# nunofonseca/fastq_utils

Measured on AMD Instinct MI355X. Metric: Mreads/s validated (fastq_info, 150bp), higher is better.
Workload: dtype u8

## Files before the change

fastq_utils_amd/csrc/fqg_mark_pack.h:

```cpp
#pragma once
#include <stdint.h>

#if defined(__HIPCC__) || defined(__CUDACC__)
#define FQG_PACK_HD __host__ __device__ inline
#else
#define FQG_PACK_HD inline
#endif

namespace fqg {

FQG_PACK_HD uint32_t udot4_u8(uint32_t a, uint32_t b, uint32_t c) {
#if defined(__HIP_DEVICE_COMPILE__)
  return __builtin_amdgcn_udot4(a, b, c, false);
#else
  for (int i = 0; i < 4; ++i) c += ((a >> (8 * i)) & 0xFFu) * ((b >> (8 * i)) & 0xFFu);
  return c;
#endif
}

FQG_PACK_HD uint32_t as_computed(uint32_t x) {
#if defined(__HIP_DEVICE_COMPILE__)
  asm("" : "+v"(x));
#endif
  return x;
}

FQG_PACK_HD uint32_t mark_pair(uint32_t m0, uint32_t m1) {
  return udot4_u8(m1, 0x80402010u, udot4_u8(m0, 0x08040201u, 0u));
}

FQG_PACK_HD uint32_t pack_marks32(uint32_t m0, uint32_t m1, uint32_t m2, uint32_t m3, uint32_t m4, uint32_t m5, uint32_t m6,
                                  uint32_t m7) {
  const uint32_t a = as_computed((mark_pair(m2, m3) << 8) | mark_pair(m0, m1));
  const uint32_t b = as_computed((mark_pair(m6, m7) << 8) | mark_pair(m4, m5));
  return (b << 9) | (a >> 7);
}

}
```

fastq_utils_amd/csrc/fqg_stream_kernels.hip:

```cpp
#include "fqg_device.h"
#include "fqg_type_spans.h"
#include "fqg_mark_pack.h"
#include "fqg_part_steps.h"
#include "fqg_line_window.h"

namespace fqg {

constexpr uint32_t kH = 0x80808080u;

__device__ __forceinline__ uint32_t pack_marks16(uint32_t m0, uint32_t m1, uint32_t m2, uint32_t m3) {
  uint32_t lo = __builtin_amdgcn_udot4(m0, 0x08040201u, 0u, false);
  lo = __builtin_amdgcn_udot4(m1, 0x80402010u, lo, false);
  uint32_t hi = __builtin_amdgcn_udot4(m2, 0x08040201u, 0u, false);
  hi = __builtin_amdgcn_udot4(m3, 0x80402010u, hi, false);
  return (lo >> 7) | (hi << 1);
}

__device__ __forceinline__ uint32_t nl_marks7(uint32_t w, uint32_t& bad) {
  const uint32_t x = w ^ 0x0A0A0A0Au;
  const uint32_t t = kH - x;
  const uint32_t c = t + 0x1F1F1F1Fu;
  bad = __builtin_amdgcn_bitop3_b32(bad, c, t, 0xF4);
  return t & kH;
}
__device__ __forceinline__ uint32_t or3(uint32_t a, uint32_t b, uint32_t c) { return __builtin_amdgcn_bitop3_b32(a, b, c, 0xFE); }

__device__ __forceinline__ uint32_t in_vgpr(uint32_t x) {
  uint32_t v;
  asm volatile("v_mov_b32 %0, %1" : "=v"(v) : "s"(x));
  return v;
}

__device__ __forceinline__ uint32_t not_acgtn7(uint32_t w) {
  const uint32_t want = __builtin_amdgcn_perm(0x474E7F54u, 0x437F417Fu, w & 0x07070707u);
  return ((w ^ want) + 0x7F7F7F7Fu) & kH;
}

__device__ __forceinline__ uint32_t in_range7(uint32_t w, uint32_t lob, uint32_t hihb, uint32_t kh = kH) {
  return ((w | kH) - lob) & (hihb - w) & kh;
}
__device__ __forceinline__ uint32_t in_range7a(uint32_t w, uint32_t lo_add, uint32_t hihb, uint32_t kh) {
  return (w + lo_add) & (hihb - w) & kh;
}

constexpr uint32_t kBootMax = 64u << 10;
constexpr int kBootBlock = 1024;
__global__ __launch_bounds__(kBootBlock) void k_stream_boot(const uint8_t* __restrict__ img, uint32_t span,
                                                            CallState* __restrict__ cs) {
  constexpr int kBootWaves = kBootBlock / kWave;
  __shared__ uint32_t s_cnt[kBootWaves];
  __shared__ __attribute__((aligned(16))) uint8_t s_img[kBootMax];
  const int lane = lane_id(), wv = threadIdx.x >> 6;
  const uint32_t part = span / kBootWaves;
  for (uint32_t o = threadIdx.x * 16u; o < span; o += kBootBlock * 16u)
    *reinterpret_cast<uint4*>(s_img + o) = *reinterpret_cast<const uint4*>(img + o);
  __syncthreads();
  const uint8_t* p = s_img + (uint64_t)wv * part;
  uint32_t cnt = 0;
  for (uint32_t o = lane; o < part; o += kWave) cnt += (p[o] == '\n');
  cnt = wave_sum(cnt);
  if (lane == 0) s_cnt[wv] = cnt;
  __syncthreads();
  uint32_t before = 0, total = 0;
  for (int w = 0; w < kBootWaves; ++w) {
    if (w < wv) before += s_cnt[w];
    total += s_cnt[w];
  }
  const uint32_t limit = total & ~3u;
  if (threadIdx.x == 0) cs->boot_lines = total;
  uint32_t line = before, qmin = 255, qmax = 0;
  for (uint32_t o = 0; o < part; o += kWave) {
    const uint32_t c = o + lane < part ? (uint32_t)p[o + lane] : 0u;
    const uint64_t bal = __ballot(o + lane < part && c == '\n');
    const uint32_t mine = line + (uint32_t)__builtin_popcountll(bal & ((1ull << lane) - 1ull));
    if ((mine & 3u) == 3u && mine < limit && c != '\n' && o + lane < part) {
      qmin = c < qmin ? c : qmin;
      qmax = c > qmax ? c : qmax;
    }
    line += (uint32_t)__builtin_popcountll(bal);
  }
#pragma unroll
  for (int d = 32; d > 0; d >>= 1) {
    const uint32_t a = __shfl_xor(qmin, d, 64), b = __shfl_xor(qmax, d, 64);
    qmin = a < qmin ? a : qmin;
    qmax = b > qmax ? b : qmax;
  }
  if (lane == 0 && qmin <= qmax) {
    atomicMin(&cs->boot_qmin, qmin);
    atomicMax(&cs->boot_qmax, qmax);
    atomicMin(&cs->qmin_byte, qmin);
    atomicMax(&cs->qmax_byte, qmax);
  }
}

struct StreamOut {
  uint32_t* counts;
  uint32_t* cinfo;
  uint16_t* stage;
  unsigned long long* queue;
  unsigned long long queue_cap;
};

__device__ __forceinline__ void queue_suspect(const StreamOut& o, CallState* cs, uint64_t pos) {
  if (__hip_atomic_load(&cs->queue_count, __ATOMIC_RELAXED, __HIP_MEMORY_SCOPE_AGENT) > o.queue_cap) return;
  const unsigned long long at = atomicAdd(&cs->queue_count, 1ull);
  if (at < o.queue_cap) o.queue[at] = pos;
}

constexpr int kHalves = 2;
constexpr int kLaneBytes = 32;
constexpr int kHalfBytes = kWave * kLaneBytes;

struct Piece32 {
  uint4 a, b;
};

constexpr uint32_t kCopyFront = 16, kCopyBack = 64;
constexpr uint32_t kCopyRow = kCopyFront + kChunkBytes + kCopyBack;

__device__ __forceinline__ uint32_t stage_entry(uint32_t ent, uint32_t c1) {
  return ent | ((c1 == '@' ? kClsAt : (c1 == '+' ? kClsPlus : 0u)) << 12);
}

template <uint32_t ABL>
__device__ __forceinline__ void stage_chunk(const uint8_t* __restrict__ img, uint64_t n, uint64_t cb, uint32_t chunk,
                                            const uint32_t (&nl)[kHalves], const uint32_t (&nl2)[kHalves],
                                            const uint32_t (&ex)[kHalves], uint32_t tot, bool fits,
                                            uint16_t* __restrict__ slots, const uint8_t* __restrict__ copy,
                                            uint32_t tail, uint16_t* __restrict__ stage, bool interior) {
  const int lane = lane_id();
#pragma unroll
  for (int k = 0; k < kHalves; ++k) {
    uint32_t m = nl[k], r = ex[k];
    const uint32_t at = (uint32_t)k * kHalfBytes + (uint32_t)lane * kLaneBytes;
    if (fits) {
      while (m) {
        const uint32_t j = (uint32_t)__builtin_ctz(m);
        m &= m - 1;
        slots[r] = (uint16_t)((__builtin_amdgcn_ubfe(nl2[k], j, 1u) << 14) | as_computed(at | j));
        ++r;
      }
      continue;
    }
    while (m) {
      const uint32_t j = (uint32_t)__builtin_ctz(m);
      m &= m - 1;
      if (r < (uint32_t)kStageCap) slots[r] = (uint16_t)((at + j) | (((nl2[k] >> j) & 1u) << 14));
      ++r;
    }
  }
  __builtin_amdgcn_wave_barrier();
  uint16_t* dst = stage + (uint64_t)chunk * kStageCap;
  for (uint32_t i = lane; i < tot; i += kWave) {
    const uint32_t ent = slots[i];
    const uint32_t o = (ent & 0xFFFu) + 1;
    uint32_t c1 = 0;
    if (!(ABL & 4u)) {
      if (interior) c1 = o < (uint32_t)kChunkBytes ? (uint32_t)copy[o] : (tail & 0xFFu);
      else c1 = cb + o < n ? (uint32_t)img[cb + o] : 0u;
    }
    dst[i] = (uint16_t)stage_entry(ent, c1);
  }
}

template <int NAMES>
struct Pass1Lds {
  uint16_t slots[kBlock / kWave][kStageCap];
  __attribute__((aligned(16))) uint8_t copy[kBlock / kWave][NAMES ? kCopyRow : (uint32_t)kChunkBytes];
};
template <uint32_t ABL, int NAMES>
__device__ __forceinline__ void stream_pass1_body(const uint8_t* __restrict__ img, uint64_t n, uint32_t n_chunks, const StreamOut& o,
                                                  CallState* __restrict__ cs, const NameCapture& nc, uint32_t block,
                                                  Pass1Lds<NAMES>& lds) {
  static_assert(kHalves == 2 && kHalves * kHalfBytes == kChunkBytes, "one packed scan covers the two slices");
  static_assert(NAMES == 0 || !(ABL & 7u), "the name capture needs the speculation, the staged entries and the copy");
  auto& s_slots = lds.slots;
  auto& s_copy = lds.copy;
  const int lane = lane_id(), wv = __builtin_amdgcn_readfirstlane((int)(threadIdx.x >> 6));
  uint8_t* const copy = s_copy[wv] + (NAMES ? kCopyFront : 0u);
  const uint32_t chunk = block * (kBlock / kWave) + wv;
  if (chunk >= n_chunks) return;
  const uint64_t cb = (uint64_t)chunk * kChunkBytes;
  const uint64_t wb = cb + (uint64_t)lane * kLaneBytes;
  const bool interior = cb + kChunkBytes + 4 <= n;
  uint32_t nl[kHalves], ex[kHalves];
  Piece32 v[kHalves];
  uint32_t flags = 0;

  uint32_t tail = 0;
  uint32_t prev = '\n';
  const uint32_t boot_lo = cs->boot_qmin, boot_hi = cs->boot_qmax;
  if (interior) {
    tail = *reinterpret_cast<const uint32_t*>(img + cb + kChunkBytes);
    if (NAMES && chunk) prev = *reinterpret_cast<const uint32_t*>(img + cb - 4) >> 24;
#pragma unroll
    for (int k = 0; k < kHalves; ++k) {
      v[k].a = *reinterpret_cast<const uint4*>(img + wb + (uint64_t)k * kHalfBytes);
      v[k].b = *reinterpret_cast<const uint4*>(img + wb + (uint64_t)k * kHalfBytes + 16);
    }
    if (!(ABL & 6u)) {
#pragma unroll
      for (int k = 0; k < kHalves; ++k) {
        *reinterpret_cast<uint4*>(&copy[k * kHalfBytes + lane * kLaneBytes]) = v[k].a;
        *reinterpret_cast<uint4*>(&copy[k * kHalfBytes + lane * kLaneBytes + 16]) = v[k].b;
      }
    }
    uint32_t hiacc = 0, badacc = 0;
#pragma unroll
    for (int k = 0; k < kHalves; ++k) {
      hiacc = or3(or3(or3(or3(hiacc, v[k].a.x, v[k].a.y), v[k].a.z, v[k].a.w), v[k].b.x, v[k].b.y), v[k].b.z, v[k].b.w);
      nl[k] = pack_marks32(nl_marks7(v[k].a.x, badacc), nl_marks7(v[k].a.y, badacc), nl_marks7(v[k].a.z, badacc), nl_marks7(v[k].a.w, badacc),
                           nl_marks7(v[k].b.x, badacc), nl_marks7(v[k].b.y, badacc), nl_marks7(v[k].b.z, badacc), nl_marks7(v[k].b.w, badacc));
    }
    const bool high = __ballot((hiacc & kH) != 0) != 0;
    const bool ctrl = __ballot((badacc & kH) != 0) != 0;
    if (high) flags |= kFlagHigh;
    if (ctrl && !high) {
      uint32_t nul = 0, cr = 0;
#pragma unroll
      for (int k = 0; k < kHalves; ++k) {
        const uint32_t w[8] = {v[k].a.x, v[k].a.y, v[k].a.z, v[k].a.w, v[k].b.x, v[k].b.y, v[k].b.z, v[k].b.w};
#pragma unroll
        for (int j = 0; j < 8; ++j) {
          nul |= eq_bytes(w[j], 0u);
          cr |= eq_bytes(w[j], 0x0D0D0D0Du);
        }
      }
      if (__ballot(nul != 0)) flags |= kFlagNul;
      if (__ballot(cr != 0)) flags |= kFlagCr;
    }
  } else {
    uint32_t bad = 0;
#pragma unroll
    for (int k = 0; k < kHalves; ++k) {
      const uint64_t off = wb + (uint64_t)k * kHalfBytes;
      nl[k] = 0;
      v[k].a = v[k].b = make_uint4(0, 0, 0, 0);
      for (uint64_t i = off; i < n && i < off + kLaneBytes; ++i) {
        const uint32_t c = img[i];
        if (c == '\n') nl[k] |= 1u << (i - off);
        else if (c == 0u) bad |= kFlagNul;
        else if (c == '\r') bad |= kFlagCr;
        else if (c >= 0x80u) bad |= kFlagHigh;
      }
    }
    if (__ballot((bad & kFlagNul) != 0)) flags |= kFlagNul;
    if (__ballot((bad & kFlagCr) != 0)) flags |= kFlagCr;
    if (__ballot((bad & kFlagHigh) != 0)) flags |= kFlagHigh;
  }

  const uint32_t c01 = __popc(nl[0]) | (__popc(nl[1]) << 16);
  const uint32_t s01 = wave_scan_incl_dpp(c01);
  const uint32_t t01 = __builtin_amdgcn_readlane(s01, 63);
  const uint32_t total = (t01 & 0xFFFFu) + (t01 >> 16);
  ex[0] = (s01 & 0xFFFFu) - (c01 & 0xFFFFu);
  ex[1] = (t01 & 0xFFFFu) + (s01 >> 16) - (c01 >> 16);
  if (total > (uint32_t)kStageCap) flags |= kFlagStageOverflow;

  uint32_t tail_nl = 0;
  if (interior) {
    tail_nl = ((tail & 0xFFu) == '\n' ? 1u : 0u) | (((tail >> 8) & 0xFFu) == '\n' ? 2u : 0u);
  } else {
    for (uint64_t i = 0; i < 2; ++i)
      if (cb + kChunkBytes + i < n && img[cb + kChunkBytes + i] == '\n') tail_nl |= 1u << i;
  }
  uint32_t nl2[kHalves], cand[kHalves];
#pragma unroll
  for (int k = 0; k < kHalves; ++k) {
    uint32_t nxt = dpp0<0x130, 0xf, 0xf>(nl[k]);
    const uint32_t first_next = (uint32_t)__builtin_amdgcn_readlane(nl[k + 1 < kHalves ? k + 1 : k], 0);
    if (lane == 63) nxt = k + 1 < kHalves ? first_next : tail_nl;
    const uint32_t n1 = __builtin_amdgcn_alignbit(nxt, nl[k], 1);
    nl2[k] = __builtin_amdgcn_alignbit(nxt, nl[k], 2);
    cand[k] = nl[k] & nl2[k] & ~n1;
  }

  const uint32_t tot = total < (uint32_t)kStageCap ? total : (uint32_t)kStageCap;

  uint32_t info = kInfoUnknown;
  bool found = false;
  uint32_t t0 = 0;
  if (!(ABL & 1u) && interior && !(flags & kFlagHigh)) {
#pragma unroll
    for (int k = 0; k < kHalves; ++k) {
      const uint64_t bal = __ballot(cand[k] != 0);
      if (!found && bal) {
        const int l = __builtin_ctzll(bal);
        const uint32_t cl = (uint32_t)__builtin_amdgcn_readlane(cand[k], l);
        const uint32_t nll = (uint32_t)__builtin_amdgcn_readlane(nl[k], l);
        const uint32_t exl = (uint32_t)__builtin_amdgcn_readlane(ex[k], l);
        const uint32_t j = (uint32_t)__builtin_ctz(cl);
        const uint32_t a = exl + __popc(nll & ((1u << j) - 1u));
        t0 = (1u - a) & 3u;
        found = true;
      }
    }
    uint32_t M1[kHalves], M3[kHalves];
    bool dense = false;
    if (found) {
      uint32_t over = 0;
#pragma unroll
      for (int k = 0; k < kHalves; ++k) over |= type_spans32(nl[k], t0 + ex[k], M1[k], M3[k]);
      dense = __ballot(over != 0) != 0;
    }
    if (found && !dense) {
      info = t0;
      uint32_t lo = boot_lo, hi = boot_hi;
      if (lo > hi || lo > 127u) {
        lo = 127u;
        hi = 0u;
      }
      const uint32_t hihb_s = ((hi & 0x7Fu) | 0x80u) * 0x01010101u;
      const uint32_t lo_add = in_vgpr((0x80u - lo) * 0x01010101u), hihb = in_vgpr(hihb_s), khv = in_vgpr(kH);
      QRange q{0x00FF00FFu, 0x00FF00FFu, 0u, 0u};
      bool any_viol = false;
#pragma unroll
      for (int k = 0; k < kHalves; ++k) {
        const uint4 &a = v[k].a, &b = v[k].b;
        const uint32_t inv = pack_marks32(not_acgtn7(a.x), not_acgtn7(a.y), not_acgtn7(a.z), not_acgtn7(a.w), not_acgtn7(b.x), not_acgtn7(b.y),
                                          not_acgtn7(b.z), not_acgtn7(b.w));
        const uint32_t bad = (ABL & 8u) ? 0u : inv & M1[k];
        if (bad) queue_suspect(o, cs, wb + (uint64_t)k * kHalfBytes + (uint32_t)__builtin_ctz(bad));
        const uint32_t okq = pack_marks32(in_range7a(a.x, lo_add, hihb, khv), in_range7a(a.y, lo_add, hihb, khv), in_range7a(a.z, lo_add, hihb, khv),
                                          in_range7a(a.w, lo_add, hihb, khv), in_range7a(b.x, lo_add, hihb, khv), in_range7a(b.y, lo_add, hihb, khv),
                                          in_range7a(b.z, lo_add, hihb, khv), in_range7a(b.w, lo_add, hihb, khv));
        const uint32_t qm = (ABL & 16u) ? 0u : M3[k];
        if (__ballot((qm & ~okq) != 0)) {
          any_viol = true;
          qrange_accum(a, qm & 0xFFFFu, q);
          qrange_accum(b, qm >> 16, q);
        }
      }
      if (any_viol) {
        uint32_t qmin = pk_min_u16(q.mn_e, q.mn_o), qmax = pk_max_u16(q.mx_e, q.mx_o);
        qmin = (qmin & 0xFFFFu) < (qmin >> 16) ? (qmin & 0xFFFFu) : (qmin >> 16);
        qmax = (qmax & 0xFFFFu) > (qmax >> 16) ? (qmax & 0xFFFFu) : (qmax >> 16);
#pragma unroll
        for (int d = 32; d > 0; d >>= 1) {
          const uint32_t x = __shfl_xor(qmin, d, 64), y = __shfl_xor(qmax, d, 64);
          qmin = x < qmin ? x : qmin;
          qmax = y > qmax ? y : qmax;
        }
        if (qmin <= qmax) info |= kInfoRange | ((qmin & 0xFFu) << 8) | ((qmax & 0xFFu) << 16);
      }
    } else if (total == 0) {
      info = kInfoOneLine;
      uint32_t lo = boot_lo, hi = boot_hi;
      if (lo > hi || lo > 127u) {
        lo = 127u;
        hi = 0u;
      }
      const uint32_t lob = lo * 0x01010101u, hihb = ((hi & 0x7Fu) | 0x80u) * 0x01010101u;
      uint32_t not_base = 0, outside = 0;
#pragma unroll
      for (int k = 0; k < kHalves; ++k) {
        const uint32_t w[8] = {v[k].a.x, v[k].a.y, v[k].a.z, v[k].a.w, v[k].b.x, v[k].b.y, v[k].b.z, v[k].b.w};
#pragma unroll
        for (int j = 0; j < 8; ++j) {
          not_base |= not_acgtn7(w[j]);
          outside |= ~in_range7(w[j], lob, hihb) & kH;
        }
      }
      if (__ballot(not_base != 0)) info |= kInfoNotBases;
      if (__ballot(outside != 0)) {
        QRange q{0x00FF00FFu, 0x00FF00FFu, 0u, 0u};
#pragma unroll
        for (int k = 0; k < kHalves; ++k) {
          qrange_accum(v[k].a, 0xFFFFu, q);
          qrange_accum(v[k].b, 0xFFFFu, q);
        }
        uint32_t qmin = pk_min_u16(q.mn_e, q.mn_o), qmax = pk_max_u16(q.mx_e, q.mx_o);
        qmin = (qmin & 0xFFFFu) < (qmin >> 16) ? (qmin & 0xFFFFu) : (qmin >> 16);
        qmax = (qmax & 0xFFFFu) > (qmax >> 16) ? (qmax & 0xFFFFu) : (qmax >> 16);
#pragma unroll
        for (int d = 32; d > 0; d >>= 1) {
          const uint32_t x = __shfl_xor(qmin, d, 64), y = __shfl_xor(qmax, d, 64);
          qmin = x < qmin ? x : qmin;
          qmax = y > qmax ? y : qmax;
        }
        if (qmin <= qmax) info |= kInfoRange | ((qmin & 0xFFu) << 8) | ((qmax & 0xFFu) << 16);
      }
    }
  }

  if (!(ABL & 2u)) {
    stage_chunk<ABL>(img, n, cb, chunk, nl, nl2, ex, tot, total <= (uint32_t)kStageCap, s_slots[wv], copy, tail, o.stage, interior);
  }
  if constexpr (NAMES == 2) {
    uint32_t hc = kNoCapture;
    if (found && total <= (uint32_t)kStageCap) {
      hc = 0;
      const uint16_t* slots = s_slots[wv];
      const bool first_is_start = prev == '\n';
      uint32_t v0 = (0u - t0) & 3u;
      if (v0 == 0u && !first_is_start) v0 = 4u;
      const uint32_t sub = (uint32_t)lane & 3u, q = (uint32_t)lane >> 2;
      const bool casava = nc.fmt == FQG_NAME_CASAVA18;
      const uint32_t pe_cut = (nc.fmt == FQG_NAME_DEFAULT && nc.is_pe) ? 1u : 0u;
      for (uint32_t base = 0; v0 + 4u * base <= tot; base += kWave / 4) {
        const uint32_t j = base + q, vv = v0 + 4u * j;
        bool is_hdr = vv <= tot;
        uint32_t at = 0;
        if (is_hdr && vv > 0) {
          at = (slots[vv - 1] & 0xFFFu) + 1u;
          is_hdr = at < (uint32_t)kChunkBytes;
        }
        hc += (uint32_t)__builtin_popcountll(__ballot(is_hdr && sub == 0u));
        if (is_hdr && j < nc.K) {
// ... 69 lines not shown
          part += oth;
          if (sub == 0u) {
            typedef unsigned long long u64x2 __attribute__((ext_vector_type(2)));
            u64x2 dg;
            dg.x = name_fin(name_seed(nlen) + part);
            dg.y = (unsigned long long)(nlen | (acct << 10) | (vv << 20) | (at_sign ? kDigestAt : 0u) | (ok ? kDigestOk : 0u));
            *reinterpret_cast<u64x2*>(nc.recs + ((uint64_t)chunk * nc.K + j) * kDigestWords) = dg;
          }
        }
      }
      if (hc >= kNoCapture) hc = kNoCapture - 1u;
    }
    if (lane == 0) nc.hcount[chunk] = (uint16_t)hc;
  }
  if constexpr (NAMES == 1) {
    uint32_t hc = kNoCapture;
    if (found && total <= (uint32_t)kStageCap) {
      hc = 0;
      const uint16_t* slots = s_slots[wv];
      const bool first_is_start = prev == '\n';
      for (uint32_t base = 0; base <= tot; base += kWave) {
        const uint32_t vv = base + (uint32_t)lane;
        bool is_hdr = vv <= tot && ((t0 + vv) & 3u) == 0u && (vv > 0 || first_is_start);
        uint32_t at = 0;
        if (is_hdr && vv > 0) {
          at = (slots[vv - 1] & 0xFFFu) + 1u;
          is_hdr = at < (uint32_t)kChunkBytes;
        }
        const unsigned long long hm = __ballot(is_hdr);
        const uint32_t j = hc + (uint32_t)__builtin_popcountll(hm & ((1ull << lane) - 1ull));
        hc += (uint32_t)__builtin_popcountll(hm);
        if (is_hdr && j < nc.K) {
          bool end_known = vv < tot, real = false;
          uint32_t len = (end_known ? (uint32_t)(slots[vv] & 0xFFFu) : (uint32_t)kChunkBytes) - at;
          unsigned long long w[kNameRecWords];
          if (end_known || cb + at + kNameRecText + 1 > n) {
#pragma unroll
            for (uint32_t k = 0; k < kNameRecWords; ++k) __builtin_memcpy(&w[k], copy + at + 8u * k - 3u, 8);
          } else {
            const uint8_t* g = img + cb + at - 3u;
            unsigned long long nlm[kNameRecWords];
#pragma unroll
            for (uint32_t k = 0; k < kNameRecWords; ++k) {
              __builtin_memcpy(&w[k], g + 8u * k, 8);
              const unsigned long long y = w[k] ^ 0x0A0A0A0A0A0A0A0Aull;
              nlm[k] = ~(((y & 0x7F7F7F7F7F7F7F7Full) + 0x7F7F7F7F7F7F7F7Full) | y | 0x7F7F7F7F7F7F7F7Full);
            }
            nlm[0] &= ~0xFFFFFFull;
            real = true;
            len = kNameRecText + 1;
#pragma unroll
            for (int k = (int)kNameRecWords - 1; k >= 0; --k)
              if (nlm[k]) {
                len = 8u * (uint32_t)k + ((uint32_t)__builtin_ctzll(nlm[k]) >> 3) - 3u;
                end_known = true;
              }
          }
          len = len > 1023u ? 1023u : len;
          const uint32_t meta = len | (vv << 10) | (end_known ? 1u << 19 : 0u) | (((w[0] >> 24) & 0xFFu) == '@' ? 1u << 20 : 0u) |
                                (real ? 1u << 21 : 0u);
          w[0] = (w[0] & 0xFFFFFFFF00000000ull) | meta;
          typedef unsigned long long u64x2 __attribute__((ext_vector_type(2)));
          u64x2* dst = reinterpret_cast<u64x2*>(nc.recs + ((uint64_t)chunk * nc.K + j) * kNameRecWords);
#pragma unroll
          for (uint32_t k = 0; k < kNameRecWords / 2; ++k) {
            u64x2 x;
            x.x = w[2 * k];
            x.y = w[2 * k + 1];
            dst[k] = x;
          }
        }
      }
      if (hc >= kNoCapture) hc = kNoCapture - 1u;
    }
    if (lane == 0) nc.hcount[chunk] = (uint16_t)hc;
  }
  if (lane == 0) {
    o.counts[chunk] = total;
    o.cinfo[chunk] = info;
    if (flags) atomicOr(&cs->flags, flags);
  }
}

template <uint32_t ABL, int NAMES = 0>
__global__ __launch_bounds__(kBlock) void k_stream_pass1(const uint8_t* __restrict__ img, uint64_t n,
                                                         uint32_t n_chunks, StreamOut o,
                                                         CallState* __restrict__ cs, NameCapture nc = NameCapture{}) {
  __shared__ Pass1Lds<NAMES> lds;
  stream_pass1_body<ABL, NAMES>(img, n, n_chunks, o, cs, nc, blockIdx.x, lds);
}

struct ChunkRanks {
  const uint32_t* counts;
  const uint32_t* local;
  const unsigned long long* span_excl;
  uint32_t n_chunks;
  __device__ __forceinline__ uint64_t rank0(uint32_t c) const { return span_excl[c / kScanSpan] + local[c]; }
};

__global__ __launch_bounds__(kBlock) void k_stream_chunks(ChunkRanks cr, const uint32_t* __restrict__ cinfo, uint64_t limit,
                                                          uint32_t* __restrict__ redo, CallState* __restrict__ cs) {
  const uint32_t c = blockIdx.x * kBlock + threadIdx.x;
  const int lane = lane_id();
  bool again = false;
  if (c < cr.n_chunks) {
    const uint64_t rank0 = cr.rank0(c);
    const uint32_t cnt = cr.counts[c], info = cinfo[c];
    if (rank0 < limit) {
      if (chunk_info_redo(info, (uint32_t)rank0) || rank0 + cnt >= limit) again = true;
      else if (chunk_info_range(info, (uint32_t)rank0)) {
        const uint32_t qlo = (info >> 8) & 0xFFu, qhi = (info >> 16) & 0xFFu;
        if (qlo < __atomic_load_n(&cs->qmin_byte, __ATOMIC_RELAXED)) atomicMin(&cs->qmin_byte, qlo);
        if (qhi > __atomic_load_n(&cs->qmax_byte, __ATOMIC_RELAXED)) atomicMax(&cs->qmax_byte, qhi);
      }
    }
  }
  __shared__ uint32_t s_cnt[kBlock / kWave], s_base;
  const unsigned long long am = __ballot(again);
  const int wv = (int)(threadIdx.x >> 6);
  if (lane == 0) s_cnt[wv] = (uint32_t)__builtin_popcountll(am);
  __syncthreads();
  if (threadIdx.x == 0) {
    uint32_t tot = 0;
#pragma unroll
    for (int w = 0; w < kBlock / kWave; ++w) tot += s_cnt[w];
    s_base = tot ? atomicAdd(&cs->redo_count, tot) : 0u;
  }
  __syncthreads();
  if (again) {
    uint32_t at = s_base + (uint32_t)__builtin_popcountll(am & ((1ull << lane) - 1ull));
    for (int w = 0; w < wv; ++w) at += s_cnt[w];
    if (at < cr.n_chunks) redo[at] = c;
  }
}

__device__ __forceinline__ uint32_t chunk_of_rank(const ChunkRanks& cr, uint64_t R, uint32_t g) {
  const uint32_t n = cr.n_chunks;
  if (g >= n) g = n - 1;
  uint32_t lo, hi, step = 1;
  if (cr.rank0(g) <= R) {
    lo = g;
    for (;;) {
      const uint32_t t = lo + step;
      if (t >= n) {
        hi = n;
        break;
      }
      if (cr.rank0(t) <= R) {
        lo = t;
        step <<= 1;
      } else {
        hi = t;
        break;
      }
    }
  } else {
    hi = g;
    for (;;) {
      const uint32_t t = hi > step ? hi - step : 0;
      if (cr.rank0(t) <= R) {
        lo = t;
        break;
      }
      hi = t;
      step <<= 1;
    }
  }
  while (hi - lo > 1) {
    const uint32_t mid = lo + (hi - lo) / 2;
    if (cr.rank0(mid) <= R) lo = mid;
    else hi = mid;
  }
// ... 441 lines not shown
      const uint32_t rl = l1 + 1;
      const unsigned long long cm = (call & kHasAcc) ? __ballot(rl <= FQG_MAX_READ_LENGTH - 1) : 0ull;
      if (cm) {
        const bool counted = rl <= FQG_MAX_READ_LENGTH - 1;
        const uint32_t rl0 = (uint32_t)__builtin_amdgcn_readlane((int)rl, __builtin_ctzll(cm));
        const unsigned long long same = __ballot(counted && rl == rl0);
        const uint32_t n_same = (uint32_t)__builtin_popcountll(same);
        if (rl0 != run_len) {
          run_flush();
          run_len = rl0;
          run_cnt = 0;
        }
        run_cnt += n_same;
        if (same != cm) {
          if (counted && rl != rl0) {
            atomicAdd(&row[kOddOk], 1u);
            atomicMin(&row[kOddMin], rl);
            atomicMax(&row[kOddMax], rl);
            if (rl < (uint32_t)kLinesHist) atomicAdd(&s_hist[rl], 1u);
            else atomicAdd(&A.hist[rl], (unsigned long long)A.weight);
          }
        }
      }
      const unsigned long long sm = (call & kSusAll) ? ~0ull : __ballot(sus);
      if (sm) {
        if (lane == 0) {
          const uint64_t w = g * 2;
          if ((uint32_t)sm) A.suspect_bits[w] = (uint32_t)sm;
          if ((uint32_t)(sm >> 32)) A.suspect_bits[w + 1] = (uint32_t)(sm >> 32);
        }
      }
    }
    __builtin_amdgcn_wave_barrier();
  }
  run_flush();
  if (!A.acc) return;
  __builtin_amdgcn_fence(__ATOMIC_ACQ_REL, "wavefront");
  __builtin_amdgcn_wave_barrier();
  unsigned long long n_ok = 0, min_rl = ~0ull, max_rl = 0;
  if (lane == 0) {
    const uint32_t odd_min = row[kOddMin], odd_max = row[kOddMax];
    const uint32_t lo = u_min < odd_min ? u_min : odd_min;
    n_ok = (unsigned long long)u_ok + row[kOddOk];
    min_rl = lo == ~0u ? ~0ull : (unsigned long long)lo;
    max_rl = u_max > odd_max ? u_max : odd_max;
    s_red[0][threadIdx.x >> 6] = n_ok;
    s_red[1][threadIdx.x >> 6] = min_rl;
    s_red[2][threadIdx.x >> 6] = max_rl;
  }
  __syncthreads();
  if (threadIdx.x == 0) {
    for (int w = 1; w < kBlock / kWave; ++w) {
      n_ok += s_red[0][w];
      min_rl = s_red[1][w] < min_rl ? s_red[1][w] : min_rl;
      max_rl = s_red[2][w] > max_rl ? s_red[2][w] : max_rl;
    }
    if (n_ok) {
      atomicAdd(&A.acc->num_rds, n_ok * A.weight);
      if (min_rl < A.acc->min_rl) atomicMin(&A.acc->min_rl, min_rl);
      if (max_rl > A.acc->max_rl) atomicMax(&A.acc->max_rl, max_rl);
    }
  }
  for (int i = threadIdx.x; i < kLinesHist; i += kBlock) {
    const uint32_t cc = s_hist[i];
    if (cc) atomicAdd(&A.hist[i], (unsigned long long)cc * A.weight);
  }
}

__global__ __launch_bounds__(kBlock) __attribute__((amdgpu_waves_per_eu(7, 8))) void k_stream_lines_fast(LinesArgs A, uint8_t* __restrict__ todo) {
  __shared__ LinesFastLds lds;
  stream_lines_fast_body(A, todo, blockIdx.x, gridDim.x, lds);
}

template <int NAMES>
__global__ __launch_bounds__(kBlock) __attribute__((amdgpu_waves_per_eu(7, 8))) void k_stream_pass1_lines(
    const uint8_t* __restrict__ img, uint64_t n, uint32_t chunk_first, uint32_t n_chunks, StreamOut o, CallState* __restrict__ cs,
    LinesArgs A, uint8_t* __restrict__ todo, uint32_t line_workers, uint32_t part , NameCapture nc) {
  union Lds {
    Pass1Lds<NAMES> p1;
    LinesFastLds lf;
  };
  __shared__ Lds lds;
  if (blockIdx.x >= line_workers) {
    stream_pass1_body<0u, NAMES>(img, n, n_chunks, o, cs, nc, chunk_first / (kBlock / kWave) + (blockIdx.x - line_workers), lds.p1);
    return;
  }
  if (__hip_atomic_load(&cs->flags, __ATOMIC_RELAXED, __HIP_MEMORY_SCOPE_AGENT) & (kFlagNul | kFlagCr | kFlagHigh | kFlagStageOverflow)) return;
  static_assert(kPartStepRanks == (uint64_t)(4 * kWave * kLinesPer), "a step of the line kernels");
  const unsigned long long R = readlane64(cs->part_newlines[part], 0), R0 = part ? readlane64(cs->part_newlines[part - 1], 0) : 0ull;
  const PartSteps ps = part_steps(R0, R, chunk_first, part ? readlane64(cs->lines_done[part - 1], 0) : 0ull);
  if (blockIdx.x == 0 && threadIdx.x == 0) {
    cs->lines_done[part] = ps.done;
    if (ps.run) cs->lines_done_steps = ps.step_hi;
  }
  if (!ps.run) return;
  A.n_newlines = R;
  A.n_lines = R;
  A.limit = R & ~3ull;
  A.cr.n_chunks = chunk_first;
  A.step_lo = ps.step_lo;
  A.step_hi = ps.step_hi;
  if (A.step_hi <= A.step_lo) return;
  stream_lines_fast_body(A, todo, blockIdx.x, line_workers, lds.lf);
}

__global__ __launch_bounds__(kBlock) void k_acc_merge(AccState* __restrict__ src, unsigned long long* __restrict__ src_hist,
                                                      AccState* __restrict__ dst, unsigned long long* __restrict__ dst_hist,
                                                      int discard) {
  __shared__ unsigned long long s_lo, s_hi;
  if (threadIdx.x == 0) {
    s_lo = src->min_rl;
    s_hi = src->max_rl;
  }
  __syncthreads();
  const unsigned long long lo = s_lo, hi = s_hi;
  if (lo <= hi)
    for (unsigned long long i = lo + (unsigned long long)blockIdx.x * kBlock + threadIdx.x; i <= hi; i += (unsigned long long)gridDim.x * kBlock) {
      const unsigned long long v = src_hist[i];
      if (v) {
        if (!discard && dst_hist) atomicAdd(&dst_hist[i], v);
        src_hist[i] = 0;
      }
    }
  if (!discard && dst && blockIdx.x == 0 && threadIdx.x == 0 && src->num_rds) {
    atomicAdd(&dst->num_rds, src->num_rds);
    atomicMin(&dst->min_rl, src->min_rl);
    atomicMax(&dst->max_rl, src->max_rl);
  }
}
__global__ void k_acc_scratch_reset(AccState* __restrict__ a) {
  a->num_rds = 0;
  a->min_rl = FQG_MAX_READ_LENGTH;
  a->max_rl = 0;
  a->min_qbyte = 255;
  a->max_qbyte = 0;
}

__global__ __launch_bounds__(kBlock) void k_suspect_list(const uint32_t* __restrict__ bits, uint64_t n_records,
                                                         unsigned long long* __restrict__ list,
                                                         unsigned long long list_cap,
                                                         unsigned long long* __restrict__ list_count,
                                                         AccState* __restrict__ acc, const CallState* __restrict__ cs) {
  const uint64_t n_words = (n_records + 31) / 32;
  const uint64_t stride = (uint64_t)gridDim.x * kBlock;
  const int lane = lane_id();
  for (uint64_t w0 = (uint64_t)blockIdx.x * kBlock + (threadIdx.x & ~63u); w0 < n_words; w0 += stride) {
    const uint64_t w = w0 + (uint64_t)lane;
    uint32_t m = w < n_words ? bits[w] : 0u;
    if (w * 32 + 32 > n_records) m &= w * 32 < n_records ? (uint32_t)((1ull << (n_records - w * 32)) - 1ull) : 0u;
    const uint32_t cnt = (uint32_t)__popc(m);
    uint32_t incl = cnt;
#pragma unroll
    for (int d = 1; d < 64; d <<= 1) {
      const uint32_t o = __shfl_up(incl, d, 64);
      if (lane >= d) incl += o;
    }
    const uint32_t total = (uint32_t)__builtin_amdgcn_readlane((int)incl, 63);
    if (!total) continue;
    unsigned long long base = 0;
    if (lane == 0) base = atomicAdd(list_count, (unsigned long long)total);
    base = ((unsigned long long)(uint32_t)__builtin_amdgcn_readfirstlane((int)(uint32_t)(base >> 32)) << 32) |
           (uint32_t)__builtin_amdgcn_readfirstlane((int)(uint32_t)base);
    unsigned long long at = base + (incl - cnt);
    while (m) {
      const uint32_t j = (uint32_t)__builtin_ctz(m);
      m &= m - 1;
      if (at < list_cap) list[at] = w * 32 + j;
// ... 35 lines not shown
```

Before: 14080.

## Pack per-byte marks into bitmasks with MFMA i8 matrix ops

Replaces the udot4-based packing of per-byte mark flags into 32-bit masks with two 16x16x64 int8 MFMA instructions per pack, using per-lane weight vectors so that each lane's result rows hold its packed bits. It is applied to the newline, base-validity and quality-range mark sets, selectable by a compile-time mask. The goal is to move packing work from VALU to the matrix unit. It also pins pass1 to 8 waves per EU, which caps register use and may cause spills, and MFMA latency plus weight setup may cost more than the dot instructions they replace.

```diff
diff --git a/fastq_utils_amd/csrc/fqg_mark_pack.h b/fastq_utils_amd/csrc/fqg_mark_pack.h
--- a/fastq_utils_amd/csrc/fqg_mark_pack.h
+++ b/fastq_utils_amd/csrc/fqg_mark_pack.h
@@ -36,4 +36,77 @@
   return (b << 9) | (a >> 7);
 }
 
+constexpr uint32_t kMarkW0 = 0xF8FCFEFFu;
+constexpr uint32_t kMarkW1 = 0x80C0E0F0u;
+
+FQG_PACK_HD void mark_weights(int lane, uint32_t (&w)[4]) {
+  const int g = lane >> 4, c = lane & 15;
+  const bool lo = c == 4 * g, hi = c == 4 * g + 1;
+  w[0] = lo ? kMarkW0 : 0u;
+  w[1] = lo ? kMarkW1 : 0u;
+  w[2] = hi ? kMarkW0 : 0u;
+  w[3] = hi ? kMarkW1 : 0u;
 }
+
+#if defined(__HIPCC__)
+typedef int mark_v4i __attribute__((ext_vector_type(4)));
+struct MarkWeights {
+  mark_v4i a;
+};
+__device__ inline MarkWeights mark_weights_of(int lane) {
+  uint32_t w[4];
+  mark_weights(lane, w);
+  MarkWeights r;
+  r.a = mark_v4i{(int)w[0], (int)w[1], (int)w[2], (int)w[3]};
+  return r;
+}
+__device__ inline uint32_t pack_marks32_mfma(const MarkWeights& W, uint32_t m0, uint32_t m1, uint32_t m2, uint32_t m3, uint32_t m4,
+                                             uint32_t m5, uint32_t m6, uint32_t m7) {
+  const mark_v4i z = {0, 0, 0, 0};
+  const mark_v4i d0 = __builtin_amdgcn_mfma_i32_16x16x64_i8(W.a, mark_v4i{(int)m0, (int)m1, (int)m2, (int)m3}, z, 0, 0, 0);
+  const mark_v4i d1 = __builtin_amdgcn_mfma_i32_16x16x64_i8(W.a, mark_v4i{(int)m4, (int)m5, (int)m6, (int)m7}, z, 0, 0, 0);
+  const uint32_t a = as_computed(((uint32_t)d0[1] << 8) | (uint32_t)d0[0]);
+  const uint32_t b = as_computed(((uint32_t)d1[1] << 8) | (uint32_t)d1[0]);
+  return (b << 9) | (a >> 7);
+}
+#endif
+#if !defined(__HIP_DEVICE_COMPILE__)
+inline int8_t mark_slot(const uint32_t (&r)[4], int j) { return (int8_t)(uint8_t)(r[j >> 2] >> (8 * (j & 3))); }
+
+inline void mfma_i32_16x16x64_i8_model(const uint32_t (&A)[64][4], const uint32_t (&B)[64][4], int32_t (&D)[64][4]) {
+  int32_t a[16][64], b[64][16];
+  for (int l = 0; l < 64; ++l)
+    for (int j = 0; j < 16; ++j) {
+      a[l & 15][16 * (l >> 4) + j] = mark_slot(A[l], j);
+      b[16 * (l >> 4) + j][l & 15] = mark_slot(B[l], j);
+    }
+  for (int l = 0; l < 64; ++l)
+    for (int r = 0; r < 4; ++r) {
+      const int row = 4 * (l >> 4) + r, col = l & 15;
+      int32_t s = 0;
+      for (int k = 0; k < 64; ++k) s += a[row][k] * b[k][col];
+      D[l][r] = s;
+    }
+}
+
+inline void pack_marks32_mfma_model(const uint32_t (&marks)[64][8], uint32_t (&out)[64]) {
+  uint32_t W[64][4], B0[64][4], B1[64][4];
+  int32_t D0[64][4], D1[64][4];
+  for (int l = 0; l < 64; ++l) {
+    mark_weights(l, W[l]);
+    for (int i = 0; i < 4; ++i) {
+      B0[l][i] = marks[l][i];
+      B1[l][i] = marks[l][4 + i];
+    }
+  }
+  mfma_i32_16x16x64_i8_model(W, B0, D0);
+  mfma_i32_16x16x64_i8_model(W, B1, D1);
+  for (int l = 0; l < 64; ++l) {
+    const uint32_t a = ((uint32_t)D0[l][1] << 8) | (uint32_t)D0[l][0];
+    const uint32_t b = ((uint32_t)D1[l][1] << 8) | (uint32_t)D1[l][0];
+    out[l] = (b << 9) | (a >> 7);
+  }
+}
+#endif
+
+}
diff --git a/fastq_utils_amd/csrc/fqg_stream_kernels.hip b/fastq_utils_amd/csrc/fqg_stream_kernels.hip
--- a/fastq_utils_amd/csrc/fqg_stream_kernels.hip
+++ b/fastq_utils_amd/csrc/fqg_stream_kernels.hip
@@ -7,6 +7,17 @@
 namespace fqg {
 
 constexpr uint32_t kH = 0x80808080u;
+
+#ifndef FQG_MFMA_MARK_SETS
+#define FQG_MFMA_MARK_SETS 7
+#endif
+constexpr uint32_t kMfmaMarkSets = FQG_MFMA_MARK_SETS;
+template <uint32_t SET>
+__device__ __forceinline__ uint32_t pack_set32(const MarkWeights& W, uint32_t m0, uint32_t m1, uint32_t m2, uint32_t m3, uint32_t m4,
+                                               uint32_t m5, uint32_t m6, uint32_t m7) {
+  if constexpr ((kMfmaMarkSets & SET) != 0) return pack_marks32_mfma(W, m0, m1, m2, m3, m4, m5, m6, m7);
+  else return pack_marks32(m0, m1, m2, m3, m4, m5, m6, m7);
+}
 
 __device__ __forceinline__ uint32_t pack_marks16(uint32_t m0, uint32_t m1, uint32_t m2, uint32_t m3) {
   uint32_t lo = __builtin_amdgcn_udot4(m0, 0x08040201u, 0u, false);
@@ -180,6 +191,7 @@
   uint8_t* const copy = s_copy[wv] + (NAMES ? kCopyFront : 0u);
   const uint32_t chunk = block * (kBlock / kWave) + wv;
   if (chunk >= n_chunks) return;
+  const MarkWeights W = mark_weights_of(lane);
   const uint64_t cb = (uint64_t)chunk * kChunkBytes;
   const uint64_t wb = cb + (uint64_t)lane * kLaneBytes;
   const bool interior = cb + kChunkBytes + 4 <= n;
@@ -209,7 +221,7 @@
 #pragma unroll
     for (int k = 0; k < kHalves; ++k) {
       hiacc = or3(or3(or3(or3(hiacc, v[k].a.x, v[k].a.y), v[k].a.z, v[k].a.w), v[k].b.x, v[k].b.y), v[k].b.z, v[k].b.w);
-      nl[k] = pack_marks32(nl_marks7(v[k].a.x, badacc), nl_marks7(v[k].a.y, badacc), nl_marks7(v[k].a.z, badacc), nl_marks7(v[k].a.w, badacc),
+      nl[k] = pack_set32<1u>(W, nl_marks7(v[k].a.x, badacc), nl_marks7(v[k].a.y, badacc), nl_marks7(v[k].a.z, badacc), nl_marks7(v[k].a.w, badacc),
                            nl_marks7(v[k].b.x, badacc), nl_marks7(v[k].b.y, badacc), nl_marks7(v[k].b.z, badacc), nl_marks7(v[k].b.w, badacc));
     }
     const bool high = __ballot((hiacc & kH) != 0) != 0;
@@ -317,11 +329,11 @@
 #pragma unroll
       for (int k = 0; k < kHalves; ++k) {
         const uint4 &a = v[k].a, &b = v[k].b;
-        const uint32_t inv = pack_marks32(not_acgtn7(a.x), not_acgtn7(a.y), not_acgtn7(a.z), not_acgtn7(a.w), not_acgtn7(b.x), not_acgtn7(b.y),
+        const uint32_t inv = pack_set32<2u>(W, not_acgtn7(a.x), not_acgtn7(a.y), not_acgtn7(a.z), not_acgtn7(a.w), not_acgtn7(b.x), not_acgtn7(b.y),
                                           not_acgtn7(b.z), not_acgtn7(b.w));
         const uint32_t bad = (ABL & 8u) ? 0u : inv & M1[k];
         if (bad) queue_suspect(o, cs, wb + (uint64_t)k * kHalfBytes + (uint32_t)__builtin_ctz(bad));
-        const uint32_t okq = pack_marks32(in_range7a(a.x, lo_add, hihb, khv), in_range7a(a.y, lo_add, hihb, khv), in_range7a(a.z, lo_add, hihb, khv),
+        const uint32_t okq = pack_set32<4u>(W, in_range7a(a.x, lo_add, hihb, khv), in_range7a(a.y, lo_add, hihb, khv), in_range7a(a.z, lo_add, hihb, khv),
                                           in_range7a(a.w, lo_add, hihb, khv), in_range7a(b.x, lo_add, hihb, khv), in_range7a(b.y, lo_add, hihb, khv),
                                           in_range7a(b.z, lo_add, hihb, khv), in_range7a(b.w, lo_add, hihb, khv));
         const uint32_t qm = (ABL & 16u) ? 0u : M3[k];
@@ -560,7 +572,7 @@
 }
 
 template <uint32_t ABL, int NAMES = 0>
-__global__ __launch_bounds__(kBlock) void k_stream_pass1(const uint8_t* __restrict__ img, uint64_t n,
+__global__ __launch_bounds__(kBlock) __attribute__((amdgpu_waves_per_eu(8, 8))) void k_stream_pass1(const uint8_t* __restrict__ img, uint64_t n,
                                                          uint32_t n_chunks, StreamOut o,
                                                          CallState* __restrict__ cs, NameCapture nc = NameCapture{}) {
   __shared__ Pass1Lds<NAMES> lds;
```

After: 13420. 0.954x the previous value.

## Pack byte marks into bitmasks with i8 MFMA in fused pass1 path

Applied to the files above, without the earlier changes.

Adds a wave-level mark packer that uses the 16x16x64 i8 MFMA instruction with per-lane constant weight tiles in place of the per-lane udot4 chains that turn byte-level newline, base and quality marks into 32-bit masks. It is enabled in the fused pass1+lines kernel and adds a host reference model. The standalone pass1 kernel also gets a waves_per_eu(8,8) occupancy hint. This moves VALU packing work onto the matrix cores, at the cost of MFMA latency, a per-lane weight load and extra registers.

```diff
diff --git a/fastq_utils_amd/csrc/fqg_mark_pack.h b/fastq_utils_amd/csrc/fqg_mark_pack.h
--- a/fastq_utils_amd/csrc/fqg_mark_pack.h
+++ b/fastq_utils_amd/csrc/fqg_mark_pack.h
@@ -36,4 +36,73 @@
   return (b << 9) | (a >> 7);
 }
 
+constexpr uint32_t kPackW0 = 0xF8FCFEFFu, kPackW1 = 0x80C0E0F0u;
+struct PackWeights {
+  uint32_t w[64][4];
+};
+constexpr PackWeights make_pack_weights() {
+  PackWeights t{};
+  for (int l = 0; l < 64; ++l) {
+    const bool mine = (l % 16) / 4 == l / 16;
+    const int r = l % 4;
+    t.w[l][0] = mine && r == 0 ? kPackW0 : 0u;
+    t.w[l][1] = mine && r == 0 ? kPackW1 : 0u;
+    t.w[l][2] = mine && r == 1 ? kPackW0 : 0u;
+    t.w[l][3] = mine && r == 1 ? kPackW1 : 0u;
+  }
+  return t;
 }
+
+#if defined(__HIPCC__)
+typedef int pack_v4i __attribute__((ext_vector_type(4)));
+__device__ const PackWeights kPackWeights = make_pack_weights();
+__device__ __forceinline__ pack_v4i pack_weights(int lane) {
+  return *reinterpret_cast<const pack_v4i*>(kPackWeights.w[lane]);
+}
+__device__ __forceinline__ uint32_t pack_marks32_wave(pack_v4i wts, uint32_t m0, uint32_t m1, uint32_t m2, uint32_t m3, uint32_t m4,
+                                                      uint32_t m5, uint32_t m6, uint32_t m7) {
+  const pack_v4i zero = {0, 0, 0, 0};
+  const pack_v4i lo = __builtin_amdgcn_mfma_i32_16x16x64_i8(wts, pack_v4i{(int)m0, (int)m1, (int)m2, (int)m3}, zero, 0, 0, 0);
+  const pack_v4i hi = __builtin_amdgcn_mfma_i32_16x16x64_i8(wts, pack_v4i{(int)m4, (int)m5, (int)m6, (int)m7}, zero, 0, 0, 0);
+  const uint32_t a = as_computed(((uint32_t)lo.y << 8) | (uint32_t)lo.x);
+  const uint32_t b = as_computed(((uint32_t)hi.y << 8) | (uint32_t)hi.x);
+  return (b << 9) | (a >> 7);
+}
+#endif
+inline void mfma_i32_16x16x64_i8_host(const uint32_t (*a)[4], const uint32_t (*b)[4], int32_t (*d)[4]) {
+  int8_t ab[64][16], bb[64][16];
+  for (int l = 0; l < 64; ++l)
+    for (int e = 0; e < 16; ++e) {
+      ab[l][e] = (int8_t)(uint8_t)(a[l][e >> 2] >> (8 * (e & 3)));
+      bb[l][e] = (int8_t)(uint8_t)(b[l][e >> 2] >> (8 * (e & 3)));
+    }
+  for (int i = 0; i < 16; ++i)
+    for (int j = 0; j < 16; ++j) {
+      int32_t sum = 0;
+      for (int g = 0; g < 4; ++g) {
+        const uint32_t* al = a[i + 16 * g];
+        if (!(al[0] | al[1] | al[2] | al[3])) continue;
+        for (int e = 0; e < 16; ++e) sum += (int32_t)ab[i + 16 * g][e] * (int32_t)bb[j + 16 * g][e];
+      }
+      d[j + 16 * (i / 4)][i % 4] = sum;
+    }
+}
+inline void pack_marks32_wave(const uint32_t (*m)[8], uint32_t* out) {
+  constexpr PackWeights wts = make_pack_weights();
+  uint32_t b_lo[64][4], b_hi[64][4];
+  int32_t lo[64][4], hi[64][4];
+  for (int l = 0; l < 64; ++l)
+    for (int w = 0; w < 4; ++w) {
+      b_lo[l][w] = m[l][w];
+      b_hi[l][w] = m[l][4 + w];
+    }
+  mfma_i32_16x16x64_i8_host(wts.w, b_lo, lo);
+  mfma_i32_16x16x64_i8_host(wts.w, b_hi, hi);
+  for (int l = 0; l < 64; ++l) {
+    const uint32_t a = ((uint32_t)lo[l][1] << 8) | (uint32_t)lo[l][0];
+    const uint32_t b = ((uint32_t)hi[l][1] << 8) | (uint32_t)hi[l][0];
+    out[l] = (b << 9) | (a >> 7);
+  }
+}
+
+}
diff --git a/fastq_utils_amd/csrc/fqg_stream_kernels.hip b/fastq_utils_amd/csrc/fqg_stream_kernels.hip
--- a/fastq_utils_amd/csrc/fqg_stream_kernels.hip
+++ b/fastq_utils_amd/csrc/fqg_stream_kernels.hip
@@ -168,7 +168,7 @@
   uint16_t slots[kBlock / kWave][kStageCap];
   __attribute__((aligned(16))) uint8_t copy[kBlock / kWave][NAMES ? kCopyRow : (uint32_t)kChunkBytes];
 };
-template <uint32_t ABL, int NAMES>
+template <uint32_t ABL, int NAMES, bool WAVE_PACK>
 __device__ __forceinline__ void stream_pass1_body(const uint8_t* __restrict__ img, uint64_t n, uint32_t n_chunks, const StreamOut& o,
                                                   CallState* __restrict__ cs, const NameCapture& nc, uint32_t block,
                                                   Pass1Lds<NAMES>& lds) {
@@ -183,6 +183,12 @@
   const uint64_t cb = (uint64_t)chunk * kChunkBytes;
   const uint64_t wb = cb + (uint64_t)lane * kLaneBytes;
   const bool interior = cb + kChunkBytes + 4 <= n;
+  pack_v4i wts = {0, 0, 0, 0};
+  if (WAVE_PACK) wts = pack_weights(lane);
+  auto pack = [&](uint32_t m0, uint32_t m1, uint32_t m2, uint32_t m3, uint32_t m4, uint32_t m5, uint32_t m6, uint32_t m7) {
+    if constexpr (WAVE_PACK) return pack_marks32_wave(wts, m0, m1, m2, m3, m4, m5, m6, m7);
+    else return pack_marks32(m0, m1, m2, m3, m4, m5, m6, m7);
+  };
   uint32_t nl[kHalves], ex[kHalves];
   Piece32 v[kHalves];
   uint32_t flags = 0;
@@ -209,8 +215,8 @@
 #pragma unroll
     for (int k = 0; k < kHalves; ++k) {
       hiacc = or3(or3(or3(or3(hiacc, v[k].a.x, v[k].a.y), v[k].a.z, v[k].a.w), v[k].b.x, v[k].b.y), v[k].b.z, v[k].b.w);
-      nl[k] = pack_marks32(nl_marks7(v[k].a.x, badacc), nl_marks7(v[k].a.y, badacc), nl_marks7(v[k].a.z, badacc), nl_marks7(v[k].a.w, badacc),
-                           nl_marks7(v[k].b.x, badacc), nl_marks7(v[k].b.y, badacc), nl_marks7(v[k].b.z, badacc), nl_marks7(v[k].b.w, badacc));
+      nl[k] = pack(nl_marks7(v[k].a.x, badacc), nl_marks7(v[k].a.y, badacc), nl_marks7(v[k].a.z, badacc), nl_marks7(v[k].a.w, badacc),
+                   nl_marks7(v[k].b.x, badacc), nl_marks7(v[k].b.y, badacc), nl_marks7(v[k].b.z, badacc), nl_marks7(v[k].b.w, badacc));
     }
     const bool high = __ballot((hiacc & kH) != 0) != 0;
     const bool ctrl = __ballot((badacc & kH) != 0) != 0;
@@ -317,13 +323,13 @@
 #pragma unroll
       for (int k = 0; k < kHalves; ++k) {
         const uint4 &a = v[k].a, &b = v[k].b;
-        const uint32_t inv = pack_marks32(not_acgtn7(a.x), not_acgtn7(a.y), not_acgtn7(a.z), not_acgtn7(a.w), not_acgtn7(b.x), not_acgtn7(b.y),
-                                          not_acgtn7(b.z), not_acgtn7(b.w));
+        const uint32_t inv = pack(not_acgtn7(a.x), not_acgtn7(a.y), not_acgtn7(a.z), not_acgtn7(a.w), not_acgtn7(b.x), not_acgtn7(b.y),
+                                  not_acgtn7(b.z), not_acgtn7(b.w));
         const uint32_t bad = (ABL & 8u) ? 0u : inv & M1[k];
         if (bad) queue_suspect(o, cs, wb + (uint64_t)k * kHalfBytes + (uint32_t)__builtin_ctz(bad));
-        const uint32_t okq = pack_marks32(in_range7a(a.x, lo_add, hihb, khv), in_range7a(a.y, lo_add, hihb, khv), in_range7a(a.z, lo_add, hihb, khv),
-                                          in_range7a(a.w, lo_add, hihb, khv), in_range7a(b.x, lo_add, hihb, khv), in_range7a(b.y, lo_add, hihb, khv),
-                                          in_range7a(b.z, lo_add, hihb, khv), in_range7a(b.w, lo_add, hihb, khv));
+        const uint32_t okq = pack(in_range7a(a.x, lo_add, hihb, khv), in_range7a(a.y, lo_add, hihb, khv), in_range7a(a.z, lo_add, hihb, khv),
+                                  in_range7a(a.w, lo_add, hihb, khv), in_range7a(b.x, lo_add, hihb, khv), in_range7a(b.y, lo_add, hihb, khv),
+                                  in_range7a(b.z, lo_add, hihb, khv), in_range7a(b.w, lo_add, hihb, khv));
         const uint32_t qm = (ABL & 16u) ? 0u : M3[k];
         if (__ballot((qm & ~okq) != 0)) {
           any_viol = true;
@@ -559,12 +565,12 @@
   }
 }
 
-template <uint32_t ABL, int NAMES = 0>
-__global__ __launch_bounds__(kBlock) void k_stream_pass1(const uint8_t* __restrict__ img, uint64_t n,
+template <uint32_t ABL, int NAMES = 0, bool WAVE_PACK = false>
+__global__ __launch_bounds__(kBlock) __attribute__((amdgpu_waves_per_eu(8, 8))) void k_stream_pass1(const uint8_t* __restrict__ img, uint64_t n,
                                                          uint32_t n_chunks, StreamOut o,
                                                          CallState* __restrict__ cs, NameCapture nc = NameCapture{}) {
   __shared__ Pass1Lds<NAMES> lds;
-  stream_pass1_body<ABL, NAMES>(img, n, n_chunks, o, cs, nc, blockIdx.x, lds);
+  stream_pass1_body<ABL, NAMES, WAVE_PACK>(img, n, n_chunks, o, cs, nc, blockIdx.x, lds);
 }
 
 struct ChunkRanks {
@@ -1172,7 +1178,7 @@
   };
   __shared__ Lds lds;
   if (blockIdx.x >= line_workers) {
-    stream_pass1_body<0u, NAMES>(img, n, n_chunks, o, cs, nc, chunk_first / (kBlock / kWave) + (blockIdx.x - line_workers), lds.p1);
+    stream_pass1_body<0u, NAMES, true>(img, n, n_chunks, o, cs, nc, chunk_first / (kBlock / kWave) + (blockIdx.x - line_workers), lds.p1);
     return;
   }
   if (__hip_atomic_load(&cs->flags, __ATOMIC_RELAXED, __HIP_MEMORY_SCOPE_AGENT) & (kFlagNul | kFlagCr | kFlagHigh | kFlagStageOverflow)) return;
```

New measurement: 13950 before, 14240 after (median of 6 runs). 2.1% higher.
